# DerEchteKarsten/RayTracer3

Measured on AMD Instinct MI355X. Metric: Mrays/s, higher is better.
Workload: dtype f32

## Files before the change

### raytracer3_amd/csrc/rt3_ctx.hpp

```cpp
#pragma once
#include <hip/hip_runtime.h>

#include <cstring>
#include <string>
#include <utility>
#include <vector>

#include "../../include/rt3.h"
#include "rt3_internal.hpp"
#include "rt3_volume.hpp"

struct ncclComm;

namespace rt3 {

inline const rt3_denoise_params kDenoiseDefaults = {5u, 7u, 0.05f, 4.0f, 0u};
inline const rt3_temporal_params kTemporalDefaults = {0.2f, 0.2f, 32u, 0.9f, 0.01f, 0u};
inline const rt3_adaptive_params kAdaptiveDefaults = {16u, 16u, 0.05f, 0.01f, 1u, 0u};
inline constexpr float kIdentity[16] = {1, 0, 0, 0, 0, 1, 0, 0, 0, 0, 1, 0, 0, 0, 0, 1};
inline void pack3x4(const float* m16, float* m12) {
    for (int col = 0; col < 4; col++)
        for (int row = 0; row < 3; row++) m12[3 * col + row] = m16[4 * col + row];
}

// ... 131 lines not shown
        uint32_t n_flat_geoms = 0, n_flat_prims = 0;
        std::vector<rt3::Placed> placed;
        uint64_t bulk_copies = 0;
        rt3::DevBuf<uint2> d_geom_mask, d_alpha;
        bool masked = false;
        uint32_t n_panes = 0, pane_first_slot = 0;
        uint32_t n_frosted = 0;
        bool marked = false;
        rt3::LbvhResult bvh;
        rt3::ShadeRecords shade;
        rt3::DevBuf<char> build_scratch;
        bool built = false;
        bool stale = false;
        uint64_t topo_gen = 0;
        uint64_t stamp = 0;
        rt3::LightTable lights;
        bool refit_planned = false;
        std::vector<rt3::RefitTree> refit_trees;
        std::vector<rt3::MeshTables> refit_tables;
        rt3::DevBuf<char> refit_scratch;
        rt3::TwoLevelState tl;
        rt3::DevBuf<unsigned long long> exit_counters;
        rt3::DevBuf<char> exit_scratch;
    } accel;

    struct Work {
        size_t cap = 0, cap_pix = 0;
        rt3::DevBuf<float> rays[2], hits, T[2];
        rt3::DevBuf<float> sh_rays, sh_contrib, lacc, radsum;
        rt3::DevBuf<float> sh2_rays, sh2_contrib, sh2_tmax;
        size_t cap_emit = 0;
        rt3::DevBuf<float> pane_dist;
        size_t cap_pane = 0;
        rt3::DevBuf<uint32_t> d_counters;
        uint32_t counters_cap = 1 << 16, counters_next = 0;
        rt3::DevBuf<unsigned long long> d_totals;
        std::vector<rt3::CounterBlock> pending_counters;
        uint64_t primary_rays_pending = 0;
        uint64_t launch_serial = 0, roulette_tested = 0, roulette_ended = 0;
    } work;

    struct Tiles {
        std::vector<rt3::PixelList> pixlists;
        std::vector<rt3::GatherLayout> gather_layouts;
        uint32_t rank = 0, n_ranks = 1, part_w = 0, part_h = 0;
        ncclComm* comm = nullptr;
        uint32_t comm_rank = 0, comm_size = 0;
        rt3::DevBuf<char> gather_buf;
    } tiles;

    struct Denoise {
        rt3_denoise_params params = rt3::kDenoiseDefaults;
        rt3::DevBuf<char> scratch;
        uint32_t variance_image = 0;
    } denoise;
    struct Temporal {
        rt3_temporal_params params = rt3::kTemporalDefaults;
        rt3_gconst prev;
        bool has_prev = false;
        uint32_t motion_image = 0;
    } temporal;
    struct Motion {
        bool dirty = false, any_moved = false, any_deformed = false;
        uint64_t stamp = 0;
        rt3::DevBuf<rt3::MotionPrevDev> d_prev;
        rt3::DevBuf<uint32_t> d_slot;
// ... 138 lines not shown
```

### raytracer3_amd/csrc/rt3_internal.hpp

```cpp
#pragma once
#include <hip/hip_runtime.h>
#include <stddef.h>
#include <stdint.h>

#include <utility>
#include <vector>

#include "rt3_camera.hpp"
#include "rt3_emit_tex.hpp"
#include "rt3_glass.hpp"
#include "rt3_math.hpp"
#include "rt3_surface.hpp"

#define RT3_FLAG_NEE_SKY 1u
#define RT3_FLAG_BLUENOISE 2u
#define RT3_FLAG_SPECULAR 4u
#define RT3_FLAG_FACEFORWARD 8u
#define RT3_FLAG_PROBE_RADIANCE 16u
#define RT3_FLAG_NEE_EMISSIVE 32u
#define RT3_FLAG_NEE_PUNCTUAL 64u

namespace rt3 {

constexpr int kExtendBlock = 256;
// ... 14 lines not shown
    kTotExtendLds = 4,
    kTotShadowLds = 5,
    kTotWords = 6
};

struct ShadeLaunch {
    GConstDev g;
    SceneDev sc;
    const uint32_t* pixels;
    const uint2* pixbn;
    uint32_t npix, width;
    FastDiv npix_div;
    uint32_t s0;
    uint32_t bounce;
    union {
        const uint4* gbuffer;
        const GlassDev* glass;
    };
    const float* depth;
    const float* in_rays;
    const float* in_hits;
    const float* in_T;
    const uint32_t* in_count;
    uint32_t n_first;
    float* out_rays;
    float* out_T;
    uint32_t* out_count;
    float* sh_rays;
    float* sh_contrib;
    uint32_t* sh_count;
    float* lacc;
    size_t stride;
    LightsDev lights;
    float* sh2_rays;
    float* sh2_contrib;
    float* sh2_tmax;
    uint32_t* sh2_count;
};
struct GeomTables {
    const float* verts;
    const uint32_t* indices;
    const FlatGeomDev* geoms;
    const uint32_t *prim_geom, *first_prim;
};

inline unsigned grid_for(uint64_t n, unsigned block, unsigned max_blocks) {
    uint64_t b = (n + block - 1) / block;
    if (b < 1) b = 1;
    return (unsigned)(b > max_blocks ? max_blocks : b);
}

void launch_raygen(hipStream_t st, const GConstDev& g, const uint32_t* pixels, uint32_t npix, float* rays, size_t stride);
void launch_gbuffer(hipStream_t st, const SceneDev& sc, const uint32_t* pixels, uint32_t npix, uint32_t width, const float* hits,
                    size_t stride, void* gbuffer, float* depth);
struct ShadeExit {
    const float4* arena = nullptr;
    uint32_t tri_off = 0, exit_off = 0;
    unsigned long long* counters = nullptr;
    uint32_t* decided = nullptr;
};
void launch_shade(hipStream_t st, bool first, ShadeLaunch L, bool punct = false, const GlassDev* glass = nullptr, bool defer = false, float* pane_dist = nullptr,
                  const ShadeExit* exit = nullptr, bool frost = false);
void launch_light(hipStream_t st, bool first, ShadeLaunch L);
void launch_pixbn(hipStream_t st, const uint32_t* pixels, uint32_t npix, const uint8_t* bluenoise, uint32_t bn_w, uint32_t bn_h, uint2* out);
void launch_accumulate(hipStream_t st, const GConstDev& g, const uint32_t* pixels, uint32_t npix, uint32_t width, const float* depth,
                       const float* lacc, size_t stride, uint32_t sb, int first_batch, int last_batch, float* radsum, void* light,
                       const void* prev);
void launch_postprocess(hipStream_t st, const GConstDev& g, const SceneDev& sc, const uint32_t* pixels, uint32_t npix, uint32_t width,
                        const float* depth, const void* in, void* out);
void launch_lens_rays(hipStream_t st, const GConstDev& g, const LensDev& lens, const uint32_t* pixels, uint32_t npix, uint32_t s0, uint32_t n_first,
                      float* rays, float* T, float* lacc, size_t stride, uint32_t* count);
void launch_lens_miss(hipStream_t st, const SceneDev& sc, const float* rays, const float* hits, float* lacc, size_t stride, uint32_t n);
void launch_accumulate_lens(hipStream_t st, const GConstDev& g, const uint32_t* pixels, uint32_t npix, uint32_t width, const float* lacc, uint32_t sb,
                            int first_batch, int last_batch, float* radsum, void* light, const void* prev);
void launch_postprocess_lens(hipStream_t st, const uint32_t* pixels, uint32_t npix, uint32_t width, const void* in, void* out);
struct GuideLaunch {
    SceneDev sc;
    const uint32_t* pixels;
    uint32_t npix, width;
    const float *rays, *hits;
    size_t stride;
    uint32_t nsb, samples;
    bool first_batch, last_batch;
    float4* img[4];
};
void launch_lens_guide(hipStream_t st, const GuideLaunch& a, uint32_t groups = 0);
constexpr uint32_t kSelftestGuideHeader = 6, kSelftestGuideRecord = 10, kSelftestGuideOut = 16;
constexpr uint32_t kSelftestLensIn = 41, kSelftestLensOut = 10;
void launch_selftest_lens(hipStream_t st, const uint32_t* in, uint32_t n, uint32_t* out);
constexpr uint32_t kSelftestGlassIn = 9, kSelftestGlassOut = 5;
void launch_selftest_glass(hipStream_t st, const uint32_t* in, uint32_t n, uint32_t* out);
constexpr uint32_t kSelftestFrostIn = 12, kSelftestFrostOut = 6;
void launch_selftest_frost(hipStream_t st, const uint32_t* in, uint32_t n, uint32_t* out);
struct RouletteLaunch;
void launch_roulette(hipStream_t st, const RouletteLaunch& a, uint32_t n_max, uint32_t groups = 0);
constexpr uint32_t kSelftestRouletteIn = 5, kSelftestRouletteOut = 5;
// ... 392 lines not shown
```

### raytracer3_amd/csrc/rt3_passes.hip

```cpp
#include <hip/hip_runtime.h>

#include <cmath>
#include <cstring>
#include <algorithm>
#include <string>
#include <vector>

#include "rt3_ctx.hpp"
#include "rt3_emit_tex.hpp"
#include "rt3_roulette.hpp"
#include "rt3_volume.hpp"

using namespace rt3;

namespace rt3 {

void motion_tables_stale(rt3_ctx* c) { c->motion.dirty = true; }

}

namespace {

uint32_t spread1by1(uint32_t x) {
    x = (x | (x << 8)) & 0x00FF00FFu;
    x = (x | (x << 4)) & 0x0F0F0F0Fu;
    x = (x | (x << 2)) & 0x33333333u;
    x = (x | (x << 1)) & 0x55555555u;
    return x;
}
uint32_t zcurve_host(uint32_t x, uint32_t y) { return spread1by1(x) | (spread1by1(y) << 1); }

void free_work(rt3_ctx* c) {
    for (int k = 0; k < 2; k++) { c->work.rays[k].reset(); c->work.T[k].reset(); }
    c->work.hits.reset(); c->work.sh_rays.reset(); c->work.sh_contrib.reset(); c->work.lacc.reset(); c->work.radsum.reset();
    c->work.sh2_rays.reset(); c->work.sh2_contrib.reset(); c->work.sh2_tmax.reset();
    c->work.cap_emit = 0;
    c->work.pane_dist.reset();
    c->work.cap_pane = 0;
    c->work.cap = 0;
    c->work.cap_pix = 0;
}
int ensure_work(rt3_ctx* c, size_t paths, size_t npix) {
    int r = RT3_OK;
    if (paths > c->work.cap) {
        size_t P = (paths + 255) & ~(size_t)255;
        c->work.cap = 0;
        for (int k = 0; k < 2 && !r; k++) {
            if (!r) r = dev_alloc(c, c->work.rays[k], 8 * P);
            if (!r) r = dev_alloc(c, c->work.T[k], 3 * P);
        }
        if (!r) r = dev_alloc(c, c->work.hits, 4 * P);
        if (!r) r = dev_alloc(c, c->work.sh_rays, 8 * P);
        if (!r) r = dev_alloc(c, c->work.sh_contrib, 2 * P);
        if (!r) r = dev_alloc(c, c->work.lacc, 4 * P);
        if (!r) c->work.cap = P;
    }
    if (!r && npix > c->work.cap_pix) {
        c->work.cap_pix = 0;
        r = dev_alloc(c, c->work.radsum, 3 * npix);
        if (!r) c->work.cap_pix = npix;
    }
    if (r) free_work(c);
    return r;
}
int ensure_emit_queue(rt3_ctx* c) {
    if (c->work.cap_emit >= c->work.cap) return RT3_OK;
    c->work.cap_emit = 0;
    int r = dev_alloc(c, c->work.sh2_rays, 8 * c->work.cap);
    if (!r) r = dev_alloc(c, c->work.sh2_contrib, 2 * c->work.cap);
    if (!r) r = dev_alloc(c, c->work.sh2_tmax, c->work.cap);
    if (!r) c->work.cap_emit = c->work.cap;
    else free_work(c);
    return r;
}

int ensure_pane_dist(rt3_ctx* c) {
    if (c->work.cap_pane >= c->work.cap) return RT3_OK;
    c->work.cap_pane = 0;
    int r = dev_alloc(c, c->work.pane_dist, c->work.cap);
    if (!r) c->work.cap_pane = c->work.cap;
    else free_work(c);
    return r;
}

int reserve_counters(rt3_ctx* c, uint32_t n, uint32_t* first) {
    if (c->work.counters_next + n > c->work.counters_cap) {
        HIPC(c, hipStreamSynchronize(c->stream));
        if (int r = harvest(c)) return r;
    }
    if (n > c->work.counters_cap) return fail(c, RT3_E_INVALID, "too many bounces x batches for the counter block");
    *first = c->work.counters_next;
    c->work.counters_next += n;
    HIPC(c, hipMemsetAsync(c->work.d_counters.get() + *first, 0, (size_t)n * 4, c->stream));
    return RT3_OK;
}
TraceLaunch ctx_trace(rt3_ctx* c) {
    TraceLaunch L;
    L.stride = c->work.cap;
    L.count = c->opt.count;
    L.totals = c->opt.count ? c->work.d_totals.get() : nullptr;
    L.alpha = alpha_dev(c);
    return L;
}
int trace_primary(rt3_ctx* c, uint32_t n) {
    uint32_t wc_slot;
    if (int r = reserve_counters(c, 1, &wc_slot)) return r;
    TraceLaunch L = ctx_trace(c);
    L.rays = c->work.rays[0].get(); L.n = n; L.work_counter = c->work.d_counters.get() + wc_slot; L.hits = c->work.hits.get();
    c->work.primary_rays_pending += n;
    ScopedTimer t(c, CAT_EXTEND);
    launch_extend(c->stream, c->accel.bvh, L);
    return RT3_OK;
}

int motion_tables(rt3_ctx* c) {
// ... 126 lines not shown
    const AbsorbDev* absorb = nullptr;
    float4* guide[4] = {nullptr, nullptr, nullptr, nullptr};
    float4* guide_prev = nullptr;
    MotionDev motion{};
    const float4* prev_pos = nullptr;
};
constexpr float kSkyDeferMinPdf = 0x1p-100f;
int path_setup(rt3_ctx* c, const rt3_gconst* g, PathSetup* ps) {
    const uint32_t B = g->bounces;
    ps->gd = gconst_dev(g);
    if (c->scene.lights.empty() || B <= 1) ps->gd.pad[0] &= ~RT3_F_NEE_PUNCTUAL;
    ps->nee = (g->pad[0] & RT3_F_NEE_SKY) && c->scene.d_sky;
    const uint32_t combo = g->pad[0] & (RT3_F_NEE_EMISSIVE | (c->scene.lights.empty() ? 0u : RT3_F_NEE_PUNCTUAL));
    if (combo && B > 1) {
        if (int r = ensure_lights(c, combo)) return r;
        ps->lights = c->accel.lights.dev();
        ps->punct = ps->lights.n != 0u && c->accel.lights.n_punct != 0u;
        if (ps->lights.n)
            if (int r = ensure_emit_queue(c)) return r;
    }
    ps->nee_e = ps->lights.n != 0u;
    ps->emit_tex = ps->nee_e && c->accel.lights.textured ? c->accel.lights.emit_tex.get() : nullptr;
    ps->sc = scene_dev(c);
    ps->defer = c->opt.defer_sky_light && ps->nee && !c->accel.has_glass && !ps->punct && ps->sc.mat_tex == nullptr && c->scene.sky_min_pdf >= kSkyDeferMinPdf;
    {
        const LbvhResult& bvh = c->accel.bvh;
        ps->shade_exit = c->opt.shade_exit_test && ps->defer && !ps->nee_e && !c->opt.count && alpha_dev(c).table == nullptr && c->accel.n_panes == 0u &&
                         bvh.exit.on && bvh.exit.off && bvh.exit.counters && bvh.layout == kLayoutWide64Q && bvh.nodes;
        if (ps->shade_exit) {
            ps->exit.arena = bvh.nodes.get();
            ps->exit.tri_off = bvh.tri_off;
            ps->exit.exit_off = bvh.exit.off;
            ps->exit.counters = bvh.exit.counters;
        }
    }
    ps->panes = c->accel.n_panes != 0u && c->accel.has_glass;
    if (ps->panes) {
        if (int r = ensure_pane_dist(c)) return r;
        ps->pane = pane_dev(c);
    }
    ps->absorb = c->accel.n_absorbing != 0u ? c->accel.d_absorb.get() : nullptr;
    ps->rr = c->roulette.on && c->roulette.params.start_bounce < B - 1u;
    ps->rr_start = c->roulette.params.start_bounce;
    ps->rr_min = c->roulette.params.min_survival;
    return RT3_OK;
}
LensDev lens_dev(const rt3_ctx* c) {
    const rt3_lens_params& p = c->lens.params;
    return LensDev{p.aperture_radius, p.focus_distance, p.pixel_jitter};
}
int roulette_begin(rt3_ctx* c, const char* pass, uint32_t samples, uint32_t bounces) {
    if (c->roulette.on && (uint64_t)samples * bounces * 8u > (1ull << 30))
        return fail(c, RT3_E_INVALID, std::string(pass) + " with roulette: samples * bounces * 8 may not exceed 2^30 (the roulette draws' RNG indices start behind it)");
    c->work.launch_serial++;
    c->work.roulette_tested = c->work.roulette_ended = 0;
    return RT3_OK;
}
int trace_batch(rt3_ctx* c, const PathSetup& ps, uint32_t W, const Resource* gb, const Resource* dp, const uint32_t* pixels, const uint2* pixbn,
                uint32_t npix, uint32_t s0, uint32_t nsb) {
    const uint32_t B = ps.gd.bounces;
    const size_t S = c->work.cap;
    const bool nee = ps.nee, nee_e = ps.nee_e;
    const uint32_t n_first = nsb * npix;
    const bool lens = ps.lens_on;
    const uint32_t n_words = (nee_e ? 6 : 4) * B;
    uint32_t first;
// ... 27 lines not shown
            launch_extend(c->stream, c->accel.bvh, tr);
        }
        if (!nee && ps.sc.sky != nullptr) {
            ScopedTimer t(c, CAT_OTHER);
            launch_lens_miss(c->stream, ps.sc, c->work.rays[0].get(), c->work.hits.get(), c->work.lacc.get(), S, n_first);
        }
        if (ps.guide[0] != nullptr) {
            GuideLaunch G{};
            G.sc = ps.sc; G.pixels = pixels; G.npix = npix; G.width = W; G.rays = c->work.rays[0].get(); G.hits = c->work.hits.get(); G.stride = S;
            G.nsb = nsb; G.samples = ps.gd.samples; G.first_batch = s0 == 0; G.last_batch = s0 + nsb >= ps.gd.samples;
            for (int k = 0; k < 4; k++) G.img[k] = ps.guide[k];
            ScopedTimer t(c, CAT_OTHER);
            launch_lens_guide(c->stream, G);
            if (ps.guide_prev != nullptr) {
                GuidePrevLaunch P{};
                P.m = ps.motion; P.prev_pos = ps.prev_pos; P.pixels = pixels; P.npix = npix; P.width = W; P.rays = G.rays; P.hits = G.hits; P.stride = S;
                P.nsb = nsb; P.samples = G.samples; P.first_batch = G.first_batch; P.last_batch = G.last_batch; P.out = ps.guide_prev;
                launch_lens_guide_prev(c->stream, P);
            }
        }
    }
    if (ps.panes) HIPC(c, hipMemsetAsync(c->work.pane_dist.get(), 0, (size_t)n_first * sizeof(float), c->stream));
    for (uint32_t bn = 0; bn < B; bn++) {
        ShadeLaunch L;
        L.g = ps.gd; L.sc = ps.sc; L.pixels = pixels; L.pixbn = pixbn; L.npix = npix; L.width = W; L.s0 = s0; L.bounce = bn;
        L.gbuffer = (const uint4*)gb->ptr; L.depth = (const float*)dp->ptr;
        L.in_rays = c->work.rays[cur].get(); L.in_hits = c->work.hits.get(); L.in_T = c->work.T[cur].get();
        L.in_count = live_cnt; L.n_first = n_first;
        L.out_rays = c->work.rays[cur ^ 1].get(); L.out_T = c->work.T[cur ^ 1].get(); L.out_count = ext_cnt_at(bn);
        L.sh_rays = c->work.sh_rays.get(); L.sh_contrib = c->work.sh_contrib.get(); L.sh_count = sh_cnt_at(bn);
        L.lacc = c->work.lacc.get(); L.stride = S;
        L.lights = ps.lights;
        L.sh2_rays = c->work.sh2_rays.get(); L.sh2_contrib = c->work.sh2_contrib.get(); L.sh2_tmax = c->work.sh2_tmax.get(); L.sh2_count = emit_cnt + bn;
        {
            ScopedTimer t(c, CAT_SHADE);
            ShadeExit sx = ps.exit;
            sx.decided = dec_cnt + bn;
            launch_shade(c->stream, bn == 0 && !lens, L, ps.punct, c->accel.has_glass ? c->accel.d_glass.get() : nullptr, ps.defer,
                         ps.panes ? c->work.pane_dist.get() : nullptr, shade_exit ? &sx : nullptr, c->accel.has_glass && c->accel.n_frosted != 0u);
        }
        cur ^= 1;
        if (nee) {
            TraceLaunch tr = ctx_trace(c);
            tr.rays = c->work.sh_rays.get(); tr.count_ptr = sh_cnt_at(bn); tr.n = n_first; tr.work_counter = pool_cur + B + bn;
            if (ps.defer) {
                tr.occluded = reinterpret_cast<uint32_t*>(c->work.sh_contrib.get()) + S;
                tr.from_root = shade_exit;
            } else {
                tr.contrib = c->work.sh_contrib.get(); tr.lacc = c->work.lacc.get();
                if (ps.panes) tr.pane = &ps.pane;
            }
            ScopedTimer t(c, CAT_SHADOW);
            launch_shadow(c->stream, c->accel.bvh, tr);
        }
        if (ps.defer) {
            ScopedTimer t(c, CAT_SHADE);
            launch_light(c->stream, bn == 0 && !lens, L);
        }
        if (nee_e && bn + 1 < B && ps.emit_tex != nullptr) {
            EmitTexLaunch E{};
            E.sc = ps.sc; E.lights = ps.lights; E.emit_tex = ps.emit_tex;
            E.rays = c->work.sh2_rays.get(); E.contrib = c->work.sh2_contrib.get(); E.count = emit_cnt + bn; E.stride = S;
            E.pixels = pixels; E.npix = npix; E.s0 = s0; E.bounces = B; E.bounce = bn; E.frame = ps.gd.frame; E.dims = ps.gd.pad[0] ? 8u : 2u;
            ScopedTimer t(c, CAT_OTHER);
            launch_emit_tex(c->stream, E, n_first);
            c->prof.stats.emit_tex_launches++;
        }
        if (nee_e && bn + 1 < B) {
            TraceLaunch tr = ctx_trace(c);
            tr.rays = c->work.sh2_rays.get(); tr.count_ptr = emit_cnt + bn; tr.n = n_first; tr.work_counter = emit_cnt + B + bn;
            tr.contrib = c->work.sh2_contrib.get(); tr.lacc = c->work.lacc.get(); tr.tmax = c->work.sh2_tmax.get();
            if (ps.panes) tr.pane = &ps.pane;
            ScopedTimer t(c, CAT_SHADOW);
            launch_shadow(c->stream, c->accel.bvh, tr);
        }
        live_cnt = ext_cnt_at(bn);
        if (rr && bn >= ps.rr_start && bn != B - 1) {
            RouletteLaunch R{};
            R.in_rays = c->work.rays[cur].get(); R.in_T = c->work.T[cur].get(); R.in_count = live_cnt;
            R.out_rays = c->work.rays[cur ^ 1].get(); R.out_T = c->work.T[cur ^ 1].get(); R.out_count = rr_cnt + bn;
            R.stride = S; R.pixels = pixels; R.npix = npix; R.s0 = s0; R.bounces = B; R.bounce = bn; R.frame = ps.gd.frame;
            R.min_survival = ps.rr_min;
            ScopedTimer t(c, CAT_OTHER);
            launch_roulette(c->stream, R, n_first);
            cur ^= 1;
            live_cnt = rr_cnt + bn;
        }
        if (bn != B - 1) {
            TraceLaunch tr = ctx_trace(c);
            tr.rays = c->work.rays[cur].get(); tr.count_ptr = live_cnt; tr.n = n_first; tr.work_counter = pool_cur + bn;
// ... 721 lines not shown
```

### raytracer3_amd/csrc/rt3_shade.hip

```cpp
#include <hip/hip_fp16.h>
#include <hip/hip_runtime.h>

#include <type_traits>

#include "rt3_bsdf.hpp"
#include "rt3_camera.hpp"
#include "rt3_glass.hpp"
#include "rt3_internal.hpp"
#include "rt3_leaf_test.hpp"
#include "rt3_math.hpp"
#include "rt3_punctual.hpp"
#include "rt3_rng.hpp"
#include "rt3_sky.hpp"
#include "rt3_surface.hpp"

namespace rt3 {

constexpr int kShadeBlock = 512;
struct BlockAppend {
    uint32_t ext, sh;
};
__device__ __forceinline__ BlockAppend block_append2(bool want_ext, bool want_sh, unsigned long long* pair ,
                                                     uint32_t* lds ) {
    constexpr int kWaves = kShadeBlock / 64;
// ... 37 lines not shown
    if (lane == 0) {
        lds[wave] = (uint32_t)__popcll(m_ext);
        lds[kW1 + wave] = (uint32_t)__popcll(m_sh);
        lds[2 * kW1 + wave] = (uint32_t)__popcll(m_sh2);
    }
    __syncthreads();
    if (threadIdx.x == 0) {
        uint32_t te = 0, ts = 0, t2 = 0;
#pragma unroll
        for (int w = 0; w < kWaves; w++) {
            const uint32_t ce = lds[w], cs = lds[kW1 + w], c2 = lds[2 * kW1 + w];
            lds[w] = te;
            lds[kW1 + w] = ts;
            lds[2 * kW1 + w] = t2;
            te += ce;
            ts += cs;
            t2 += c2;
        }
        unsigned long long old = 0ull;
        if (te | ts) old = atomicAdd(pair, (unsigned long long)te | ((unsigned long long)ts << 32));
        lds[kWaves] = (uint32_t)old;
        lds[kW1 + kWaves] = (uint32_t)(old >> 32);
        lds[2 * kW1 + kWaves] = t2 ? atomicAdd(count2, t2) : 0u;
    }
    __syncthreads();
    const unsigned long long below = (1ull << lane) - 1ull;
    BlockAppend3 r;
    r.ext = lds[kWaves] + lds[wave] + (uint32_t)__popcll(m_ext & below);
    r.sh = lds[kW1 + kWaves] + lds[kW1 + wave] + (uint32_t)__popcll(m_sh & below);
    r.sh2 = lds[2 * kW1 + kWaves] + lds[2 * kW1 + wave] + (uint32_t)__popcll(m_sh2 & below);
    return r;
}

__device__ __forceinline__ bool light_next(const ShadeLaunch& a, uint32_t it, uint32_t n, uint32_t n_round, uint32_t& held, uint32_t& i, bool& active) {
    constexpr int kWaves = kShadeBlock / 64;
    __shared__ uint32_t packed[2 * kShadeBlock];
    __shared__ uint32_t wave_count[kWaves];
    const uint32_t* src = reinterpret_cast<const uint32_t*>(a.sh_contrib);
    const uint32_t* occluded = src + a.stride;
    bool keep = false;
    uint32_t s = 0;
    if (it < n) {
        keep = occluded[it] == 0u;
        s = src[it];
    }
    const uint32_t lane = __lane_id(), wave = threadIdx.x >> 6;
    const unsigned long long m = __ballot(keep);
    if (lane == 0) wave_count[wave] = (uint32_t)__popcll(m);
    __syncthreads();
    uint32_t before = 0, total = 0;
#pragma unroll
    for (int w = 0; w < kWaves; w++) {
        const uint32_t c = wave_count[w];
        before += (uint32_t)w < wave ? c : 0u;
        total += c;
    }
    if (keep) packed[held + before + (uint32_t)__popcll(m & ((1ull << lane) - 1ull))] = s;
    held += total;
    __syncthreads();
    if (held < (uint32_t)kShadeBlock && !(it >= n_round && held != 0u)) return false;
    const uint32_t take = held < (uint32_t)kShadeBlock ? held : (uint32_t)kShadeBlock;
    active = threadIdx.x < take;
    i = active ? packed[threadIdx.x] : 0u;
    held -= take;
    if (threadIdx.x < held) packed[threadIdx.x] = packed[kShadeBlock + threadIdx.x];
    return true;
}

constexpr int shade_waves(bool mat) { return mat ? 4 : 6; }
template <bool FIRST, bool GLDS, bool EMIT = false, bool MAT = false>
__global__ __launch_bounds__(kShadeBlock) __attribute__((amdgpu_waves_per_eu(shade_waves(MAT), shade_waves(MAT)))) void k_shade(ShadeLaunch a) {
    constexpr bool PUNCT = false, GLASS = false, DEFER = false, LIGHT = false;
    constexpr bool PANE = false, EXIT = false, FROST = false;
    float* const pane_dist = nullptr;
    const ShadeExit x = {};
#include "rt3_shade_body.inc"
}
template <bool FIRST, bool GLDS, bool MAT>
__global__ __launch_bounds__(kShadeBlock) __attribute__((amdgpu_waves_per_eu(shade_waves(true), shade_waves(true)))) void k_shade_punct(ShadeLaunch a) {
    constexpr bool EMIT = true, PUNCT = true, GLASS = false, DEFER = false, LIGHT = false;
    constexpr bool PANE = false, EXIT = false, FROST = false;
    float* const pane_dist = nullptr;
    const ShadeExit x = {};
#include "rt3_shade_body.inc"
}
template <bool GLDS, bool EMIT, bool MAT, bool PUNCT>
__global__ __launch_bounds__(kShadeBlock) __attribute__((amdgpu_waves_per_eu(shade_waves(true), shade_waves(true)))) void k_shade_glass(ShadeLaunch a) {
    constexpr bool FIRST = false, GLASS = true, DEFER = false, LIGHT = false;
    constexpr bool PANE = false, EXIT = false, FROST = false;
    float* const pane_dist = nullptr;
    const ShadeExit x = {};
#include "rt3_shade_body.inc"
}
template <bool GLDS, bool EMIT, bool MAT, bool PUNCT>
__global__ __launch_bounds__(kShadeBlock) __attribute__((amdgpu_waves_per_eu(shade_waves(true), shade_waves(true)))) void k_shade_pane(ShadeLaunch a, float* pane_dist) {
    constexpr bool FIRST = false, GLASS = true, DEFER = false, LIGHT = false, PANE = true, EXIT = false, FROST = false;
    const ShadeExit x = {};
#include "rt3_shade_body.inc"
}
template <bool EMIT, bool MAT, bool PUNCT, bool PANE>
__global__ __launch_bounds__(kShadeBlock) __attribute__((amdgpu_waves_per_eu(shade_waves(true), shade_waves(true)))) void k_shade_frost(ShadeLaunch a, float* pane_dist) {
    constexpr bool FIRST = false, GLDS = false, GLASS = true, DEFER = false, LIGHT = false, EXIT = false, FROST = true;
    const ShadeExit x = {};
#include "rt3_shade_body.inc"
}
template <bool FIRST, bool GLDS, bool EMIT>
__global__ __launch_bounds__(kShadeBlock) __attribute__((amdgpu_waves_per_eu(shade_waves(false), shade_waves(false)))) void k_shade_defer(ShadeLaunch a) {
    constexpr bool MAT = false, PUNCT = false, GLASS = false, DEFER = true, LIGHT = false;
    constexpr bool PANE = false, EXIT = false, FROST = false;
    float* const pane_dist = nullptr;
    const ShadeExit x = {};
#include "rt3_shade_body.inc"
}
template <bool FIRST, bool GLDS>
__global__ __launch_bounds__(kShadeBlock) __attribute__((amdgpu_waves_per_eu(shade_waves(false), shade_waves(false)))) void k_shade_defer_exit(ShadeLaunch a, ShadeExit x) {
    constexpr bool EMIT = false, MAT = false, PUNCT = false, GLASS = false, DEFER = true, LIGHT = false;
    constexpr bool PANE = false, EXIT = true, FROST = false;
    float* const pane_dist = nullptr;
#include "rt3_shade_body.inc"
}
template <bool FIRST, bool GLDS>
__global__ __launch_bounds__(kShadeBlock) __attribute__((amdgpu_waves_per_eu(shade_waves(false), shade_waves(false)))) void k_light(ShadeLaunch a) {
    constexpr bool EMIT = false, MAT = false, PUNCT = false, GLASS = false, DEFER = false, LIGHT = true;
    constexpr bool PANE = false, EXIT = false, FROST = false;
    float* const pane_dist = nullptr;
    const ShadeExit x = {};
#include "rt3_shade_body.inc"
}
__global__ void k_selftest_glass(const uint32_t* __restrict__ in, uint32_t n, uint32_t* __restrict__ out) {
    const uint32_t i = blockIdx.x * blockDim.x + threadIdx.x;
    if (i >= n) return;
    const uint32_t* p = in + kSelftestGlassIn * (size_t)i;
    auto F = [](uint32_t u) { return __uint_as_float(u); };
    const GlassEvent e = glass_sample(F(p[0]), p[1] != 0u, v3(F(p[2]), F(p[3]), F(p[4])), v3(F(p[5]), F(p[6]), F(p[7])), F(p[8]));
    uint32_t* o = out + kSelftestGlassOut * (size_t)i;
    o[0] = e.transmit;
    o[1] = __float_as_uint(e.dir.x); o[2] = __float_as_uint(e.dir.y); o[3] = __float_as_uint(e.dir.z);
    o[4] = __float_as_uint(e.F);
}
__global__ void k_selftest_frost(const uint32_t* __restrict__ in, uint32_t n, uint32_t* __restrict__ out) {
    const uint32_t i = blockIdx.x * blockDim.x + threadIdx.x;
    if (i >= n) return;
    const uint32_t* p = in + kSelftestFrostIn * (size_t)i;
    auto F = [](uint32_t u) { return __uint_as_float(u); };
    const V3 d = v3(F(p[2]), F(p[3]), F(p[4])), nn = v3(F(p[5]), F(p[6]), F(p[7]));
    FrostEvent e;
    if (F(p[8]) > 0.0f) {
        e = frost_sample(F(p[0]), p[1] != 0u, d, nn, F(p[8]), F(p[9]), F(p[10]), F(p[11]));
    } else {
        const GlassEvent g = glass_sample(F(p[0]), p[1] != 0u, d, nn, F(p[9]));
        e.event = g.transmit;
        e.dir = g.dir;
        e.F = g.F;
        e.weight = 1.0f;
    }
    uint32_t* o = out + kSelftestFrostOut * (size_t)i;
    o[0] = e.event;
// ... 60 lines not shown
    if (defer && exit != nullptr && a.lights.n == 0u) {
        dispatch_shade(first, glds, false, false, false, [&](auto f, auto g, auto, auto, auto) {
            hipLaunchKernelGGL((k_shade_defer_exit<decltype(f)::value, decltype(g)::value>), dim3(grid), dim3(kShadeBlock), 0, st, a, *exit);
        });
        return;
    }
    if (defer) {
        dispatch_shade(first, glds, a.lights.n != 0u, false, false, [&](auto f, auto g, auto e, auto, auto) {
            hipLaunchKernelGGL((k_shade_defer<decltype(f)::value, decltype(g)::value, decltype(e)::value>), dim3(grid), dim3(kShadeBlock), 0, st, a);
        });
        return;
    }
    dispatch_shade(first, glds, a.lights.n != 0u, a.sc.mat_tex != nullptr, punct && a.lights.n != 0u, [&](auto f, auto g, auto e, auto m, auto p) {
        if constexpr (!decltype(f)::value) {
            if (glass != nullptr) {
                a.glass = glass;
                if (frost) {
                    if (pane_dist != nullptr) hipLaunchKernelGGL((k_shade_frost<decltype(e)::value, decltype(m)::value, decltype(p)::value, true>), dim3(grid), dim3(kShadeBlock), 0, st, a, pane_dist);
                    else hipLaunchKernelGGL((k_shade_frost<decltype(e)::value, decltype(m)::value, decltype(p)::value, false>), dim3(grid), dim3(kShadeBlock), 0, st, a, pane_dist);
                    return;
                }
                if (pane_dist != nullptr) {
                    hipLaunchKernelGGL((k_shade_pane<decltype(g)::value, decltype(e)::value, decltype(m)::value, decltype(p)::value>), dim3(grid), dim3(kShadeBlock), 0, st, a, pane_dist);
                    return;
                }
                hipLaunchKernelGGL((k_shade_glass<decltype(g)::value, decltype(e)::value, decltype(m)::value, decltype(p)::value>), dim3(grid), dim3(kShadeBlock), 0, st, a);
                return;
            }
        }
        if constexpr (decltype(p)::value) hipLaunchKernelGGL((k_shade_punct<decltype(f)::value, decltype(g)::value, decltype(m)::value>), dim3(grid), dim3(kShadeBlock), 0, st, a);
        else hipLaunchKernelGGL((k_shade<decltype(f)::value, decltype(g)::value, decltype(e)::value, decltype(m)::value>), dim3(grid), dim3(kShadeBlock), 0, st, a);
    });
}
void launch_light(hipStream_t st, bool first, ShadeLaunch a) {
    a.npix_div = make_fastdiv(a.npix);
    const unsigned grid = grid_for(a.n_first, kShadeBlock * 8, 8192);
    const bool glds = a.sc.shade_geoms != nullptr && a.sc.n_geoms <= kShadeGeomsLds;
    dispatch_shade(first, glds, false, false, false, [&](auto f, auto g, auto, auto, auto) {
        hipLaunchKernelGGL((k_light<decltype(f)::value, decltype(g)::value>), dim3(grid), dim3(kShadeBlock), 0, st, a);
    });
}
void launch_selftest_glass(hipStream_t st, const uint32_t* in, uint32_t n, uint32_t* out) {
    hipLaunchKernelGGL(k_selftest_glass, dim3((n + 255) / 256), dim3(256), 0, st, in, n, out);
}
void launch_selftest_frost(hipStream_t st, const uint32_t* in, uint32_t n, uint32_t* out) {
    hipLaunchKernelGGL(k_selftest_frost, dim3((n + 255) / 256), dim3(256), 0, st, in, n, out);
}
void launch_accumulate(hipStream_t st, const GConstDev& g, const uint32_t* pixels, uint32_t npix, uint32_t width, const float* depth,
                       const float* lacc, size_t stride, uint32_t sb, int first_batch, int last_batch, float* radsum, void* light,
                       const void* prev) {
    hipLaunchKernelGGL(k_accumulate, dim3(grid_for(npix, 256, 8192)), dim3(256), 0, st, g, pixels, npix, width, depth, lacc, stride, sb,
                       first_batch, last_batch, radsum, (float4*)light, (const float4*)prev);
}

}
```

### raytracer3_amd/csrc/rt3_shade_body.inc

```
    static_assert(GLASS || !FROST, "a frosted geometry is a glass geometry");
    static_assert(GLASS || !PANE, "a pane is a glass geometry");
    static_assert(!(DEFER && LIGHT) && !((DEFER || LIGHT) && (MAT || PUNCT || GLASS)), "deferral covers the plain opaque instances");
    static_assert(!(FIRST && MAT), "the first vertex is read from the G-buffer");
    static_assert(EMIT || !PUNCT, "punctual lights are records of the emitter table");
    static_assert(!(FIRST && GLASS), "the G-buffer has no room for a material class: glass frames start from camera rays");
    static_assert(!EXIT || (DEFER && !EMIT), "the exit test decides deferred sky shadow rays, in frames without an emitter queue");
    __shared__ uint32_t append_lds[2][(EMIT ? 3 : 2) * (kShadeBlock / 64 + 1)];
    __shared__ ShadeGeomDev s_geoms[GLDS ? kShadeGeomsLds : 1];
    __shared__ MatTexDev s_mats[GLDS && MAT ? kShadeGeomsLds : 1];
    __shared__ GlassDev s_glass[GLDS && GLASS ? kShadeGeomsLds : 1];
    if (GLDS) {
        const uint32_t ng = a.sc.n_geoms < kShadeGeomsLds ? a.sc.n_geoms : kShadeGeomsLds;
        const uint32_t words = ng * (uint32_t)(sizeof(ShadeGeomDev) / 4);
        for (uint32_t k = threadIdx.x; k < words; k += kShadeBlock) reinterpret_cast<uint32_t*>(s_geoms)[k] = reinterpret_cast<const uint32_t*>(a.sc.shade_geoms)[k];
        if constexpr (MAT)
            for (uint32_t k = threadIdx.x; k < ng * 4u; k += kShadeBlock) reinterpret_cast<uint32_t*>(s_mats)[k] = reinterpret_cast<const uint32_t*>(a.sc.mat_tex)[k];
        if constexpr (GLASS)
            for (uint32_t k = threadIdx.x; k < ng * 4u; k += kShadeBlock) reinterpret_cast<uint32_t*>(s_glass)[k] = reinterpret_cast<const uint32_t*>(a.glass)[k];
        __syncthreads();
    }
    uint32_t parity = 0;
    bool exit_every = false;
    uint32_t exit_tested = 0u, exit_decided = 0u;
    ExitHeader xh = {};
    if constexpr (EXIT) {
        const unsigned long long tried = x.counters[0], occluded = x.counters[1];
        exit_every = tried < kExitWarmupTries || 4ull * occluded >= tried;
        xh = *reinterpret_cast<const ExitHeader*>(reinterpret_cast<const char*>(x.arena) + x.exit_off);
    }
    constexpr uint32_t kMargRows = 2048;
    __shared__ uint32_t s_guide_marg[kMargRows];
    __shared__ float s_cdf_marg[kMargRows + 4];
    const bool marg_in_lds = (a.g.pad[0] & RT3_FLAG_NEE_SKY) && a.sc.sky != nullptr && a.sc.sky_h <= kMargRows;
    if (marg_in_lds) {
        for (uint32_t k = threadIdx.x; k < a.sc.sky_h; k += kShadeBlock) s_guide_marg[k] = a.sc.guide_marg[k];
        for (uint32_t k = threadIdx.x; k < a.sc.sky_h + 4u; k += kShadeBlock) s_cdf_marg[k] = a.sc.cdf_marg[k];
        __syncthreads();
    }
    const float* cdf_marg = marg_in_lds ? s_cdf_marg : a.sc.cdf_marg;
    const uint32_t* guide_marg = marg_in_lds ? s_guide_marg : a.sc.guide_marg;
    const GConstDev& g = a.g;
    const uint32_t flags = g.pad[0], B = g.bounces, b = a.bounce;
    const uint32_t dims = flags ? 8u : 2u;
    const bool nee = (flags & RT3_FLAG_NEE_SKY) && a.sc.sky != nullptr;
    const bool bnz = (flags & RT3_FLAG_BLUENOISE) && a.sc.bluenoise != nullptr;
    const bool spec = (flags & RT3_FLAG_SPECULAR) != 0u;
    const size_t S = a.stride;
    const uint32_t n = LIGHT ? *a.sh_count : FIRST ? a.n_first : *a.in_count;
    const uint32_t n_round = (n + (kShadeBlock - 1)) & ~(uint32_t)(kShadeBlock - 1);
    uint32_t light_held = 0;
    for (uint32_t it = blockIdx.x * blockDim.x + threadIdx.x; it < n_round + (LIGHT ? gridDim.x * blockDim.x : 0u); it += gridDim.x * blockDim.x) {
        uint32_t i = it;
        bool active = i < n;
        const bool exit_trip = EXIT && (exit_every || ((it / kShadeBlock) & 31u) == 0u);
        bool x_tested = false, x_decided = false;
        uint32_t x_entry = kEmptySlot;
        if constexpr (LIGHT) {
            if (!light_next(a, it, n, n_round, light_held, i, active)) continue;
        }
        uint32_t pid = 0;
        V3 o = v3(0, 0, 0), d = v3(0, 0, 1), T = v3(1, 1, 1);
        float t = 0.0f, pdf_b = 0.0f;
        Surface surf;
        surf.albedo = surf.emissive = v3(0, 0, 0);
        surf.normal = v3(0, 0, 1);
        surf.roughness = 1.0f;
        surf.metalness = 0.0f;
        uint32_t px = 0, py = 0, sample_in_batch = 0, bn = 0;
        HitRecord hrecord;
        hrecord.rec = make_uint4(0u, 0u, 0u, 0u);
        hrecord.prim = 0u;
        float hbu = 0.0f, hbv = 0.0f;
        uint32_t htan = 0u;
        float4 ro = make_float4(0.0f, 0.0f, 0.0f, 0.0f), rd = make_float4(0.0f, 0.0f, 1.0f, 0.0f);
        if (!FIRST && active) {
            ro = reinterpret_cast<const float4*>(a.in_rays)[i];
            rd = reinterpret_cast<const float4*>(a.in_rays)[S + i];
        }
        if (active) {
            pid = FIRST ? i : __float_as_uint(rd.w);
            sample_in_batch = fast_div(a.npix_div, pid);
            const uint2 pb = a.pixbn[pid - sample_in_batch * a.npix];
            px = pb.x & 0xFFFFu;
            py = pb.x >> 16;
            bn = pb.y;
        }
        if (FIRST) {
            if (active) {
                size_t pi = (size_t)py * a.width + px;
                float d0 = a.depth[pi];
                if (!LIGHT && d0 == kBackgroundDepth) {
                    reinterpret_cast<float4*>(a.lacc)[pid] = make_float4(0.0f, 0.0f, 0.0f, 0.0f);
                    active = false;
                } else {
                    surf = gbuffer_unpack(a.gbuffer[pi]);
                    primary_ray(g, px, py, o, d);
                    t = d0;
                }
            }
        } else if (active) {
            o = v3(ro.x, ro.y, ro.z);
            d = v3(rd.x, rd.y, rd.z);
            T = v3(a.in_T[i], a.in_T[S + i], a.in_T[2 * S + i]);
            pdf_b = ro.w;
            const float4 hrec = reinterpret_cast<const float4*>(a.in_hits)[i];
            uint32_t prim = __float_as_uint(hrec.w);
            if (!LIGHT && prim == kMiss) {
                if (nee && pdf_b > 0.0f) {
                    float su, sv;
                    direction_to_equirect_uv(d, su, sv);
                    float pl;
                    V3 rad = sky_eval_and_pdf(a.sc, su, sv, pl);
                    float w = pdf_b / (pdf_b + pl);
                    float4* Lp = reinterpret_cast<float4*>(a.lacc) + pid;
                    float4 lv = *Lp;
                    *Lp = make_float4(lv.x + T.x * (rad.x * w), lv.y + T.y * (rad.y * w), lv.z + T.z * (rad.z * w), 0.0f);
                }
                if constexpr (GLASS) {
                    if (!nee && b != 0u && pdf_b == kFloatMax && a.sc.sky != nullptr) {
                        float su, sv;
                        direction_to_equirect_uv(d, su, sv);
                        const V3 rad = sky_eval(a.sc, su, sv);
                        float4* Lp = reinterpret_cast<float4*>(a.lacc) + pid;
                        float4 lv = *Lp;
                        *Lp = make_float4(lv.x + T.x * rad.x, lv.y + T.y * rad.y, lv.z + T.z * rad.z, 0.0f);
                    }
                }
                active = false;
            } else {
                t = hrec.x;
                hbu = hrec.y;
                hbv = hrec.z;
                hrecord = hit_fetch(a.sc, prim);
                if constexpr (MAT) htan = tan_fetch(a.sc, prim);
            }
        }
        bool emit_shadow = false, emit_ext = false;
        V3 wl = v3(0, 1, 0), contrib = v3(0, 0, 0), nd = v3(0, 0, 1), Tn = T;
        float pdf_n = 0.0f;
        float dist_n = 0.0f;
        bool emit_shadow_e = false;
        V3 wle = v3(0, 1, 0), contrib_e = v3(0, 0, 0);
        float tmax_e = 0.0f;
        if (active) {
            uint32_t seed = rng_seed(px, py, g.frame);
            uint32_t sm = a.s0 + sample_in_batch;
            uint32_t base = (sm * B + b) * dims;
            float u0 = uniform_float(seed, base), u1 = uniform_float(seed, base + 1);
            if (bnz) {
                u0 = bluenoise_shift(u0, bn & 0xFFu);
                u1 = bluenoise_shift(u1, (bn >> 8) & 0xFFu);
            }
            V3 rad = v3(0.0f, 0.0f, 0.0f);
            float pl = 0.0f, cosl = 0.0f;
            SkyPick pick;
            pick.u = pick.v = pick.sin_theta = 0.0f;
            pick.x = pick.y = 0;
            if (nee) {
                float ul0 = uniform_float(seed, base + 3), ul1 = uniform_float(seed, base + 4);
                if (bnz) {
                    ul0 = bluenoise_shift(ul0, (bn >> 16) & 0xFFu);
                    ul1 = bluenoise_shift(ul1, (bn >> 24) & 0xFFu);
                }
                pick = sky_sample_direction(a.sc, cdf_marg, guide_marg, ul0, ul1, wl);
            }
            const bool nee_e = !LIGHT && EMIT && b + 1u < B;
// ... 220 lines not shown
            exit_tested += (uint32_t)__popcll(__ballot(x_tested));
            exit_decided += (uint32_t)__popcll(__ballot(x_decided));
        }
        if constexpr (LIGHT) {
            if (emit_shadow) {
                float4* Lp = reinterpret_cast<float4*>(a.lacc) + pid;
                float4 v = *Lp;
                *Lp = make_float4(v.x + contrib.x, v.y + contrib.y, v.z + contrib.z, 0.0f);
            }
            continue;
        }
        BlockAppend slot;
        uint32_t slot_e = 0;
        if (EMIT) {
            const BlockAppend3 s3 = block_append3(emit_ext, emit_shadow, emit_shadow_e, reinterpret_cast<unsigned long long*>(a.out_count), a.sh2_count, append_lds[parity]);
            slot.ext = s3.ext;
            slot.sh = s3.sh;
            slot_e = s3.sh2;
        } else {
            slot = block_append2(emit_ext, emit_shadow, reinterpret_cast<unsigned long long*>(a.out_count), append_lds[parity]);
        }
        parity ^= 1u;
        if (EMIT && emit_shadow_e) {
            reinterpret_cast<float4*>(a.sh2_rays)[slot_e] = make_float4(o.x, o.y, o.z, contrib_e.x);
            reinterpret_cast<float4*>(a.sh2_rays)[S + slot_e] = make_float4(wle.x, wle.y, wle.z, contrib_e.y);
            reinterpret_cast<float2*>(a.sh2_contrib)[slot_e] = make_float2(contrib_e.z, __uint_as_float(pid));
            a.sh2_tmax[slot_e] = tmax_e;
        }
        if (DEFER && emit_shadow) {
            const uint32_t j = slot.sh;
            reinterpret_cast<float4*>(a.sh_rays)[j] = make_float4(o.x, o.y, o.z, kRayTMin);
            reinterpret_cast<float4*>(a.sh_rays)[S + j] = make_float4(wl.x, wl.y, wl.z, kBackgroundDepth);
            reinterpret_cast<uint32_t*>(a.sh_contrib)[j] = i;
        } else if (emit_shadow) {
            const uint32_t j = slot.sh;
            reinterpret_cast<float4*>(a.sh_rays)[j] = make_float4(o.x, o.y, o.z, contrib.x);
            reinterpret_cast<float4*>(a.sh_rays)[S + j] = make_float4(wl.x, wl.y, wl.z, contrib.y);
            reinterpret_cast<float2*>(a.sh_contrib)[j] = make_float2(contrib.z, __uint_as_float(pid));
        }
        if (emit_ext) {
            const uint32_t j = slot.ext;
            reinterpret_cast<float4*>(a.out_rays)[j] = make_float4(o.x, o.y, o.z, pdf_n);
            reinterpret_cast<float4*>(a.out_rays)[S + j] = make_float4(nd.x, nd.y, nd.z, __uint_as_float(pid));
            a.out_T[j] = Tn.x;
            a.out_T[S + j] = Tn.y;
            a.out_T[2 * S + j] = Tn.z;
            if (PANE) pane_dist[pid] = dist_n;
        }
    }
    if constexpr (EXIT) {
        __shared__ uint32_t s_exit[2 * (kShadeBlock / 64)];
        if (__lane_id() == 0u) {
            s_exit[threadIdx.x >> 6] = exit_tested;
            s_exit[kShadeBlock / 64 + (threadIdx.x >> 6)] = exit_decided;
        }
        __syncthreads();
        if (threadIdx.x == 0u) {
            unsigned long long nt = 0ull, nd = 0ull;
            for (int w = 0; w < kShadeBlock / 64; w++) {
                nt += s_exit[w];
                nd += s_exit[kShadeBlock / 64 + w];
            }
            if (nt) atomicAdd(&x.counters[0], nt);
            if (nd) {
                atomicAdd(&x.counters[1], nd);
                atomicAdd(x.decided, (uint32_t)nd);
// ... 4 lines not shown
```

Measured before the change: 8681.

## Compact light-pass inputs into shadow-slot-indexed records from the deferred exit shade

Result: no change. 8692, median of 6 (+0.1%).

```diff
diff --git a/raytracer3_amd/csrc/rt3_ctx.hpp b/raytracer3_amd/csrc/rt3_ctx.hpp
--- a/raytracer3_amd/csrc/rt3_ctx.hpp
+++ b/raytracer3_amd/csrc/rt3_ctx.hpp
@@ -187,6 +187,10 @@
         size_t cap_emit = 0;
         rt3::DevBuf<float> pane_dist;
         size_t cap_pane = 0;
+        rt3::DevBuf<char> light_rec;
+        float4 *rec_dir = nullptr, *rec_T = nullptr;
+        float2* rec_uv = nullptr;
+        size_t cap_rec = 0;
         rt3::DevBuf<uint32_t> d_counters;
         uint32_t counters_cap = 1 << 16, counters_next = 0;
         rt3::DevBuf<unsigned long long> d_totals;
diff --git a/raytracer3_amd/csrc/rt3_internal.hpp b/raytracer3_amd/csrc/rt3_internal.hpp
--- a/raytracer3_amd/csrc/rt3_internal.hpp
+++ b/raytracer3_amd/csrc/rt3_internal.hpp
@@ -70,9 +70,18 @@
     float* lacc;
     size_t stride;
     LightsDev lights;
-    float* sh2_rays;
-    float* sh2_contrib;
-    float* sh2_tmax;
+    union {
+        float* sh2_rays;
+        float4* rec_dir;
+    };
+    union {
+        float* sh2_contrib;
+        float4* rec_T;
+    };
+    union {
+        float* sh2_tmax;
+        float2* rec_uv;
+    };
     uint32_t* sh2_count;
 };
 struct GeomTables {
@@ -99,7 +108,7 @@
 };
 void launch_shade(hipStream_t st, bool first, ShadeLaunch L, bool punct = false, const GlassDev* glass = nullptr, bool defer = false, float* pane_dist = nullptr,
                   const ShadeExit* exit = nullptr, bool frost = false);
-void launch_light(hipStream_t st, bool first, ShadeLaunch L);
+void launch_light(hipStream_t st, bool first, ShadeLaunch L, bool rec = false);
 void launch_pixbn(hipStream_t st, const uint32_t* pixels, uint32_t npix, const uint8_t* bluenoise, uint32_t bn_w, uint32_t bn_h, uint2* out);
 void launch_accumulate(hipStream_t st, const GConstDev& g, const uint32_t* pixels, uint32_t npix, uint32_t width, const float* depth,
                        const float* lacc, size_t stride, uint32_t sb, int first_batch, int last_batch, float* radsum, void* light,
diff --git a/raytracer3_amd/csrc/rt3_passes.hip b/raytracer3_amd/csrc/rt3_passes.hip
--- a/raytracer3_amd/csrc/rt3_passes.hip
+++ b/raytracer3_amd/csrc/rt3_passes.hip
@@ -37,6 +37,10 @@
     c->work.cap_emit = 0;
     c->work.pane_dist.reset();
     c->work.cap_pane = 0;
+    c->work.light_rec.reset();
+    c->work.rec_dir = c->work.rec_T = nullptr;
+    c->work.rec_uv = nullptr;
+    c->work.cap_rec = 0;
     c->work.cap = 0;
     c->work.cap_pix = 0;
 }
@@ -81,6 +85,21 @@
     if (!r) c->work.cap_pane = c->work.cap;
     else free_work(c);
     return r;
+}
+
+int ensure_light_records(rt3_ctx* c) {
+    if (c->work.cap_rec >= c->work.cap) return RT3_OK;
+    c->work.cap_rec = 0;
+    BufLayout plan;
+    plan.add(&c->work.rec_dir, c->work.cap).add(&c->work.rec_T, c->work.cap).add(&c->work.rec_uv, c->work.cap);
+    hipError_t e = c->work.light_rec.alloc_bytes(plan.bytes());
+    if (e == hipSuccess) e = plan.carve(c->work.light_rec);
+    if (e != hipSuccess) {
+        free_work(c);
+        HIPC(c, e);
+    }
+    c->work.cap_rec = c->work.cap;
+    return RT3_OK;
 }
 
 int reserve_counters(rt3_ctx* c, uint32_t n, uint32_t* first) {
@@ -273,6 +292,7 @@
             ps->exit.tri_off = bvh.tri_off;
             ps->exit.exit_off = bvh.exit.off;
             ps->exit.counters = bvh.exit.counters;
+            if (int r = ensure_light_records(c)) return r;
         }
     }
     ps->panes = c->accel.n_panes != 0u && c->accel.has_glass;
@@ -366,6 +386,8 @@
         L.lacc = c->work.lacc.get(); L.stride = S;
         L.lights = ps.lights;
         L.sh2_rays = c->work.sh2_rays.get(); L.sh2_contrib = c->work.sh2_contrib.get(); L.sh2_tmax = c->work.sh2_tmax.get(); L.sh2_count = emit_cnt + bn;
+        const bool light_rec = shade_exit && !(bn == 0 && !lens);
+        if (light_rec) { L.rec_dir = c->work.rec_dir; L.rec_T = c->work.rec_T; L.rec_uv = c->work.rec_uv; }
         {
             ScopedTimer t(c, CAT_SHADE);
             ShadeExit sx = ps.exit;
@@ -389,7 +411,7 @@
         }
         if (ps.defer) {
             ScopedTimer t(c, CAT_SHADE);
-            launch_light(c->stream, bn == 0 && !lens, L);
+            launch_light(c->stream, bn == 0 && !lens, L, light_rec);
         }
         if (nee_e && bn + 1 < B && ps.emit_tex != nullptr) {
             EmitTexLaunch E{};
diff --git a/raytracer3_amd/csrc/rt3_shade.hip b/raytracer3_amd/csrc/rt3_shade.hip
--- a/raytracer3_amd/csrc/rt3_shade.hip
+++ b/raytracer3_amd/csrc/rt3_shade.hip
@@ -93,6 +93,7 @@
     return r;
 }
 
+template <bool REC = false>
 __device__ __forceinline__ bool light_next(const ShadeLaunch& a, uint32_t it, uint32_t n, uint32_t n_round, uint32_t& held, uint32_t& i, bool& active) {
     constexpr int kWaves = kShadeBlock / 64;
     __shared__ uint32_t packed[2 * kShadeBlock];
@@ -103,7 +104,7 @@
     uint32_t s = 0;
     if (it < n) {
         keep = occluded[it] == 0u;
-        s = src[it];
+        s = REC ? it : src[it];
     }
     const uint32_t lane = __lane_id(), wave = threadIdx.x >> 6;
     const unsigned long long m = __ballot(keep);
@@ -132,7 +133,7 @@
 template <bool FIRST, bool GLDS, bool EMIT = false, bool MAT = false>
 __global__ __launch_bounds__(kShadeBlock) __attribute__((amdgpu_waves_per_eu(shade_waves(MAT), shade_waves(MAT)))) void k_shade(ShadeLaunch a) {
     constexpr bool PUNCT = false, GLASS = false, DEFER = false, LIGHT = false;
-    constexpr bool PANE = false, EXIT = false, FROST = false;
+    constexpr bool PANE = false, EXIT = false, FROST = false, REC = false;
     float* const pane_dist = nullptr;
     const ShadeExit x = {};
 #include "rt3_shade_body.inc"
@@ -140,7 +141,7 @@
 template <bool FIRST, bool GLDS, bool MAT>
 __global__ __launch_bounds__(kShadeBlock) __attribute__((amdgpu_waves_per_eu(shade_waves(true), shade_waves(true)))) void k_shade_punct(ShadeLaunch a) {
     constexpr bool EMIT = true, PUNCT = true, GLASS = false, DEFER = false, LIGHT = false;
-    constexpr bool PANE = false, EXIT = false, FROST = false;
+    constexpr bool PANE = false, EXIT = false, FROST = false, REC = false;
     float* const pane_dist = nullptr;
     const ShadeExit x = {};
 #include "rt3_shade_body.inc"
@@ -148,27 +149,27 @@
 template <bool GLDS, bool EMIT, bool MAT, bool PUNCT>
 __global__ __launch_bounds__(kShadeBlock) __attribute__((amdgpu_waves_per_eu(shade_waves(true), shade_waves(true)))) void k_shade_glass(ShadeLaunch a) {
     constexpr bool FIRST = false, GLASS = true, DEFER = false, LIGHT = false;
-    constexpr bool PANE = false, EXIT = false, FROST = false;
+    constexpr bool PANE = false, EXIT = false, FROST = false, REC = false;
     float* const pane_dist = nullptr;
     const ShadeExit x = {};
 #include "rt3_shade_body.inc"
 }
 template <bool GLDS, bool EMIT, bool MAT, bool PUNCT>
 __global__ __launch_bounds__(kShadeBlock) __attribute__((amdgpu_waves_per_eu(shade_waves(true), shade_waves(true)))) void k_shade_pane(ShadeLaunch a, float* pane_dist) {
-    constexpr bool FIRST = false, GLASS = true, DEFER = false, LIGHT = false, PANE = true, EXIT = false, FROST = false;
+    constexpr bool FIRST = false, GLASS = true, DEFER = false, LIGHT = false, PANE = true, EXIT = false, FROST = false, REC = false;
     const ShadeExit x = {};
 #include "rt3_shade_body.inc"
 }
 template <bool EMIT, bool MAT, bool PUNCT, bool PANE>
 __global__ __launch_bounds__(kShadeBlock) __attribute__((amdgpu_waves_per_eu(shade_waves(true), shade_waves(true)))) void k_shade_frost(ShadeLaunch a, float* pane_dist) {
-    constexpr bool FIRST = false, GLDS = false, GLASS = true, DEFER = false, LIGHT = false, EXIT = false, FROST = true;
+    constexpr bool FIRST = false, GLDS = false, GLASS = true, DEFER = false, LIGHT = false, EXIT = false, FROST = true, REC = false;
     const ShadeExit x = {};
 #include "rt3_shade_body.inc"
 }
 template <bool FIRST, bool GLDS, bool EMIT>
 __global__ __launch_bounds__(kShadeBlock) __attribute__((amdgpu_waves_per_eu(shade_waves(false), shade_waves(false)))) void k_shade_defer(ShadeLaunch a) {
     constexpr bool MAT = false, PUNCT = false, GLASS = false, DEFER = true, LIGHT = false;
-    constexpr bool PANE = false, EXIT = false, FROST = false;
+    constexpr bool PANE = false, EXIT = false, FROST = false, REC = false;
     float* const pane_dist = nullptr;
     const ShadeExit x = {};
 #include "rt3_shade_body.inc"
@@ -176,14 +177,22 @@
 template <bool FIRST, bool GLDS>
 __global__ __launch_bounds__(kShadeBlock) __attribute__((amdgpu_waves_per_eu(shade_waves(false), shade_waves(false)))) void k_shade_defer_exit(ShadeLaunch a, ShadeExit x) {
     constexpr bool EMIT = false, MAT = false, PUNCT = false, GLASS = false, DEFER = true, LIGHT = false;
-    constexpr bool PANE = false, EXIT = true, FROST = false;
+    constexpr bool PANE = false, EXIT = true, FROST = false, REC = false;
     float* const pane_dist = nullptr;
 #include "rt3_shade_body.inc"
 }
 template <bool FIRST, bool GLDS>
 __global__ __launch_bounds__(kShadeBlock) __attribute__((amdgpu_waves_per_eu(shade_waves(false), shade_waves(false)))) void k_light(ShadeLaunch a) {
     constexpr bool EMIT = false, MAT = false, PUNCT = false, GLASS = false, DEFER = false, LIGHT = true;
-    constexpr bool PANE = false, EXIT = false, FROST = false;
+    constexpr bool PANE = false, EXIT = false, FROST = false, REC = false;
+    float* const pane_dist = nullptr;
+    const ShadeExit x = {};
+#include "rt3_shade_body.inc"
+}
+template <bool GLDS>
+__global__ __launch_bounds__(kShadeBlock) __attribute__((amdgpu_waves_per_eu(shade_waves(false), shade_waves(false)))) void k_light_rec(ShadeLaunch a) {
+    constexpr bool FIRST = false, EMIT = false, MAT = false, PUNCT = false, GLASS = false, DEFER = false, LIGHT = true;
+    constexpr bool PANE = false, EXIT = false, FROST = false, REC = true;
     float* const pane_dist = nullptr;
     const ShadeExit x = {};
 #include "rt3_shade_body.inc"
@@ -310,10 +319,15 @@
         else hipLaunchKernelGGL((k_shade<decltype(f)::value, decltype(g)::value, decltype(e)::value, decltype(m)::value>), dim3(grid), dim3(kShadeBlock), 0, st, a);
     });
 }
-void launch_light(hipStream_t st, bool first, ShadeLaunch a) {
+void launch_light(hipStream_t st, bool first, ShadeLaunch a, bool rec) {
     a.npix_div = make_fastdiv(a.npix);
     const unsigned grid = grid_for(a.n_first, kShadeBlock * 8, 8192);
     const bool glds = a.sc.shade_geoms != nullptr && a.sc.n_geoms <= kShadeGeomsLds;
+    if (rec && !first) {
+        if (glds) hipLaunchKernelGGL(k_light_rec<true>, dim3(grid), dim3(kShadeBlock), 0, st, a);
+        else hipLaunchKernelGGL(k_light_rec<false>, dim3(grid), dim3(kShadeBlock), 0, st, a);
+        return;
+    }
     dispatch_shade(first, glds, false, false, false, [&](auto f, auto g, auto, auto, auto) {
         hipLaunchKernelGGL((k_light<decltype(f)::value, decltype(g)::value>), dim3(grid), dim3(kShadeBlock), 0, st, a);
     });
diff --git a/raytracer3_amd/csrc/rt3_shade_body.inc b/raytracer3_amd/csrc/rt3_shade_body.inc
--- a/raytracer3_amd/csrc/rt3_shade_body.inc
+++ b/raytracer3_amd/csrc/rt3_shade_body.inc
@@ -19,6 +19,7 @@
             for (uint32_t k = threadIdx.x; k < ng * 4u; k += kShadeBlock) reinterpret_cast<uint32_t*>(s_glass)[k] = reinterpret_cast<const uint32_t*>(a.glass)[k];
         __syncthreads();
     }
+    __shared__ float4 s_rec[EXIT && !FIRST ? 2 * kShadeBlock : 1];
     uint32_t parity = 0;
     bool exit_every = false;
     uint32_t exit_tested = 0u, exit_decided = 0u;
@@ -56,7 +57,7 @@
         bool x_tested = false, x_decided = false;
         uint32_t x_entry = kEmptySlot;
         if constexpr (LIGHT) {
-            if (!light_next(a, it, n, n_round, light_held, i, active)) continue;
+            if (!light_next<REC>(a, it, n, n_round, light_held, i, active)) continue;
         }
         uint32_t pid = 0;
         V3 o = v3(0, 0, 0), d = v3(0, 0, 1), T = v3(1, 1, 1);
@@ -73,7 +74,9 @@
         float hbu = 0.0f, hbv = 0.0f;
         uint32_t htan = 0u;
         float4 ro = make_float4(0.0f, 0.0f, 0.0f, 0.0f), rd = make_float4(0.0f, 0.0f, 1.0f, 0.0f);
-        if (!FIRST && active) {
+        if constexpr (LIGHT && REC) {
+            if (active) rd = a.rec_dir[i];
+        } else if (!FIRST && active) {
             ro = reinterpret_cast<const float4*>(a.in_rays)[i];
             rd = reinterpret_cast<const float4*>(a.in_rays)[S + i];
         }
@@ -101,9 +104,17 @@
         } else if (active) {
             o = v3(ro.x, ro.y, ro.z);
             d = v3(rd.x, rd.y, rd.z);
-            T = v3(a.in_T[i], a.in_T[S + i], a.in_T[2 * S + i]);
-            pdf_b = ro.w;
-            const float4 hrec = reinterpret_cast<const float4*>(a.in_hits)[i];
+            float4 hrec;
+            if constexpr (LIGHT && REC) {
+                const float4 rt = a.rec_T[i];
+                const float2 uv = a.rec_uv[i];
+                T = v3(rt.x, rt.y, rt.z);
+                hrec = make_float4(0.0f, uv.x, uv.y, rt.w);
+            } else {
+                T = v3(a.in_T[i], a.in_T[S + i], a.in_T[2 * S + i]);
+                pdf_b = ro.w;
+                hrec = reinterpret_cast<const float4*>(a.in_hits)[i];
+            }
             uint32_t prim = __float_as_uint(hrec.w);
             if (!LIGHT && prim == kMiss) {
                 if (nee && pdf_b > 0.0f) {
@@ -132,6 +143,10 @@
                 hbu = hrec.y;
                 hbv = hrec.z;
                 hrecord = hit_fetch(a.sc, prim);
+                if constexpr (EXIT && !FIRST) {
+                    s_rec[threadIdx.x] = make_float4(rd.x, rd.y, rd.z, T.x);
+                    s_rec[kShadeBlock + threadIdx.x] = make_float4(T.y, T.z, hbu, hbv);
+                }
                 if constexpr (MAT) htan = tan_fetch(a.sc, prim);
             }
         }
@@ -418,6 +433,12 @@
             reinterpret_cast<float4*>(a.sh_rays)[j] = make_float4(o.x, o.y, o.z, kRayTMin);
             reinterpret_cast<float4*>(a.sh_rays)[S + j] = make_float4(wl.x, wl.y, wl.z, kBackgroundDepth);
             reinterpret_cast<uint32_t*>(a.sh_contrib)[j] = i;
+            if constexpr (EXIT && !FIRST) {
+                const float4 q0 = s_rec[threadIdx.x], q1 = s_rec[kShadeBlock + threadIdx.x];
+                a.rec_dir[j] = make_float4(q0.x, q0.y, q0.z, __uint_as_float(pid));
+                a.rec_T[j] = make_float4(q0.w, q1.x, q1.y, a.in_hits[4 * (size_t)i + 3]);
+                a.rec_uv[j] = make_float2(q1.z, q1.w);
+            }
         } else if (emit_shadow) {
             const uint32_t j = slot.sh;
             reinterpret_cast<float4*>(a.sh_rays)[j] = make_float4(o.x, o.y, o.z, contrib.x);
```
